# biuyq/CT-GAN

Hardware: AMD Instinct MI355X
Metric: img/s per (n_critic D + 1 G) step, CIFAR-10 ResNet (higher is better)
Workload: dtype f32

## Files before the change

ctgan_amd/csrc/fewch.hip:

```cpp
#include <hip/hip_runtime.h>
#include <stdint.h>
#include <stdlib.h>

#include "common.h"

namespace {

constexpr int NT = 256;

typedef float f32x2 __attribute__((ext_vector_type(2)));
__device__ __forceinline__ f32x2 pkfma(f32x2 a, f32x2 b, f32x2 c) { return __builtin_elementwise_fma(a, b, c); }
struct Acc4 { f32x2 lo, hi; };
__device__ __forceinline__ void fma4(float s, const Acc4& w, Acc4& a) {
    const f32x2 sv = {s, s};
    a.lo = pkfma(sv, w.lo, a.lo); a.hi = pkfma(sv, w.hi, a.hi);
}
__device__ __forceinline__ float4 to_f4(const Acc4& a) { return make_float4(a.lo.x, a.lo.y, a.hi.x, a.hi.y); }
__device__ __forceinline__ Acc4 to_acc(const float4& v) { Acc4 a; a.lo = f32x2{v.x, v.y}; a.hi = f32x2{v.z, v.w}; return a; }

template <int CTRL>
__device__ __forceinline__ float dpp_add(float v) {
    const int t = __builtin_amdgcn_update_dpp(0, __builtin_bit_cast(int, v), CTRL, 0xF, 0xF, true);
    return v + __builtin_bit_cast(float, t);
}
// ... 200 lines not shown
        const int c = i & 127, tj = i >> 7, j = tj % JS, t = tj / JS;
        wbuf[i] = p.w[p.w_off + (t / 3) * p.ws_r + (t % 3) * p.ws_s + (long long)c * p.ws_c + j * p.ws_j];
    }
    __builtin_amdgcn_s_waitcnt(0xF70 | 0);
    __syncthreads();
    f32x2 wlo[9][JS], whi[9][JS];
#pragma unroll
    for (int t = 0; t < 9; ++t)
#pragma unroll
        for (int j = 0; j < JS; ++j) {
            const float4 q = *reinterpret_cast<const float4*>(&wbuf[(t * JS + j) * 128 + l * 4]);
            wlo[t][j] = f32x2{q.x, q.y}; whi[t][j] = f32x2{q.z, q.w};
        }
    __builtin_amdgcn_sched_barrier(0);
    const int LPR = W >> 4;
    const float* img = p.x + (long long)n * p.xs_n;
    auto issue_row = [&](int r) {
        const int slot = (r + 1) & (RING_SLOTS - 1);
        if (r < 0 || r >= H) {
            for (int i = tid; i < W * 32; i += RING_NT) tile4[slot * slot_f4 + 32 + i] = zero4;
            return;
        }
        if (p.dbg & 1) return;
        const float* rowp = img + (long long)r * p.xs_h + (lane & 31) * 4;
        for (int c = 0; c < LPR; ++c) {
            const int chunk = c * 8 + wave;
            const unsigned dst = (unsigned)((slot * slot_f4 + (1 + 2 * chunk) * 32) * 16);
            lds_load16(rowp + (long long)(2 * chunk + (lane >> 5)) * p.xs_w, __builtin_amdgcn_readfirstlane(dst));
        }
    };
    const int last_row = p0 + np;
    for (int r = p0 - 1; r <= p0 + RING_AHEAD && r <= last_row; ++r) issue_row(r);

    for (int pp = 0; pp < np; ++pp) {
        const int prow = p0 + pp;
        if (prow + 1 + RING_AHEAD <= last_row) issue_row(prow + 1 + RING_AHEAD);
        int after = 0;
        for (int r = prow + 2; r <= prow + 1 + RING_AHEAD && r <= last_row; ++r) after += (r >= 0 && r < H) ? LPR : 0;
        wait_vmcnt(after);
        __syncthreads();
        const float4* r0 = tile4 + ((prow + 0) & (RING_SLOTS - 1)) * slot_f4;
        const float4* r1 = tile4 + ((prow + 1) & (RING_SLOTS - 1)) * slot_f4;
        const float4* r2 = tile4 + ((prow + 2) & (RING_SLOTS - 1)) * slot_f4;
        for (int qc = grp; qc < W && !(p.dbg & 2); qc += 16) {
            f32x2 acc[JS];
#pragma unroll
            for (int j = 0; j < JS; ++j) acc[j] = f32x2{0.f, 0.f};
#pragma unroll
            for (int r = 0; r < 3; ++r) {
                const float4* rowp = r == 0 ? r0 : (r == 1 ? r1 : r2);
#pragma unroll
                for (int s2 = 0; s2 < 3; ++s2) {
                    float4 xv = rowp[(qc + s2) * 32 + l];
                    if (p.relu_in) { xv.x = fmaxf(xv.x, 0.f); xv.y = fmaxf(xv.y, 0.f); xv.z = fmaxf(xv.z, 0.f); xv.w = fmaxf(xv.w, 0.f); }
                    const f32x2 xlo = {xv.x, xv.y}, xhi = {xv.z, xv.w};
#pragma unroll
                    for (int j = 0; j < JS; ++j) acc[j] = pkfma(xhi, whi[r * 3 + s2][j], pkfma(xlo, wlo[r * 3 + s2][j], acc[j]));
                }
            }
#pragma unroll
            for (int j = 0; j < JS; ++j) {
                float v = row16_sum(acc[j].x + acc[j].y);
                v += __shfl_xor(v, 16, 64);
                if (l == 0) obuf[(pp * JS + j) * W + qc] = v;
            }
        }
    }
    __syncthreads();
    for (int i = tid; i < np * JS * W; i += RING_NT) {
        const int qc = i % W, j = (i / W) % JS, pp = i / (W * JS);
        p.y[n * p.ys_n + (long long)j * p.ys_c + (long long)(p0 + pp) * p.ys_p + (long long)qc * p.ys_q] = obuf[i] + (p.bias ? p.bias[j] : 0.f);
    }
}


struct PXParams {
    const float* x; long long xs_n, xs_h, xs_w; int H, CM;
    float* y; long long ys_n, ys_c, ys_p, ys_q;
    const float* w; long long w_off, ws_r, ws_s, ws_c, ws_j;
    const float* bias;
    int relu_in, tiles;
    const float* bn_mean; const float* bn_rstd; const float* bn_scale; const float* bn_offset; int bn_per, tanh_out;
};
constexpr int PX_TH = 8, PX_W = 32, PX_CC = 32, PX_PS = 36, PX_NT = 256;
constexpr int PX_PIX = (PX_TH + 2) * (PX_W + 2);
constexpr int PX_F4 = PX_PIX * (PX_CC / 4);
constexpr int PX_PF = (PX_F4 + PX_NT - 1) / PX_NT;

template <int JS>
__global__ __launch_bounds__(PX_NT) void m2f_px_kernel(const PXParams p) {
    extern __shared__ __attribute__((aligned(16))) float tile[];
    float4* wl = reinterpret_cast<float4*>(tile + PX_PIX * PX_PS);
    constexpr int WF4 = 9 * (PX_CC / 4) * JS;
    static_assert(WF4 <= PX_NT, "one filter float4 per thread");
    const int tid = threadIdx.x;
    const int n = blockIdx.x / p.tiles, tb = blockIdx.x - n * p.tiles;
    const int p0 = tb * PX_TH;
    const int row = tid >> 5, col = tid & 31;
    const float* img = p.x + (long long)n * p.xs_n;
    float4 pf[PX_PF], wpf = make_float4(0.f, 0.f, 0.f, 0.f);
    auto fetch = [&](int chunk) {
        float4 mu = make_float4(0.f, 0.f, 0.f, 0.f), rs = mu, ga = mu, be = mu;
        if (p.bn_mean) {
            const int c = chunk * PX_CC + (tid & 7) * 4, g = n / p.bn_per;
            mu = *reinterpret_cast<const float4*>(p.bn_mean + (long long)g * p.CM + c); rs = *reinterpret_cast<const float4*>(p.bn_rstd + (long long)g * p.CM + c);
            ga = *reinterpret_cast<const float4*>(p.bn_scale + c); be = *reinterpret_cast<const float4*>(p.bn_offset + c);
        }
#pragma unroll
        for (int k = 0; k < PX_PF; ++k) {
            const int i = tid + k * PX_NT;
            const int pix = i >> 3, c4 = i & 7;
            const int tr = pix / (PX_W + 2), tw = pix - tr * (PX_W + 2);
            const int ih = p0 - 1 + tr, iw = tw - 1;
            float4 v = make_float4(0.f, 0.f, 0.f, 0.f);
            if (i < PX_F4 && (unsigned)ih < (unsigned)p.H && (unsigned)iw < (unsigned)PX_W) {
                v = *reinterpret_cast<const float4*>(img + (long long)ih * p.xs_h + (long long)iw * p.xs_w + chunk * PX_CC + c4 * 4);
                if (p.bn_mean) {
                    v.x = (v.x - mu.x) * rs.x * ga.x + be.x; v.y = (v.y - mu.y) * rs.y * ga.y + be.y;
                    v.z = (v.z - mu.z) * rs.z * ga.z + be.z; v.w = (v.w - mu.w) * rs.w * ga.w + be.w;
                }
            }
            pf[k] = v;
        }
        if (tid < WF4) {
            const int j = tid % JS, tc = tid / JS, c4 = tc & 7, t = tc >> 3;
            const float* q = p.w + p.w_off + (t / 3) * p.ws_r + (t % 3) * p.ws_s + (long long)(chunk * PX_CC + c4 * 4) * p.ws_c + j * p.ws_j;
            wpf = make_float4(q[0], q[p.ws_c], q[2 * p.ws_c], q[3 * p.ws_c]);
        }
    };
    auto stash = [&]() {
#pragma unroll
        for (int k = 0; k < PX_PF; ++k) {
            const int i = tid + k * PX_NT;
            if (i < PX_F4) {
                float4 v = pf[k];
                if (p.relu_in) { v.x = fmaxf(v.x, 0.f); v.y = fmaxf(v.y, 0.f); v.z = fmaxf(v.z, 0.f); v.w = fmaxf(v.w, 0.f); }
                *reinterpret_cast<float4*>(&tile[(i >> 3) * PX_PS + (i & 7) * 4]) = v;
            }
        }
        if (tid < WF4) wl[tid] = wpf;
    };
    f32x2 acc[JS][2];
#pragma unroll
    for (int j = 0; j < JS; ++j) { acc[j][0] = f32x2{0.f, 0.f}; acc[j][1] = f32x2{0.f, 0.f}; }
    const int nchunk = p.CM / PX_CC;
    fetch(0);
    for (int chunk = 0; chunk < nchunk; ++chunk) {
        __syncthreads();
        stash();
        __syncthreads();
        if (chunk + 1 < nchunk) fetch(chunk + 1);
#pragma unroll
        for (int t = 0; t < 9; ++t) {
            const int r = t / 3, s2 = t % 3;
            const float* xp = &tile[((row + r) * (PX_W + 2) + col + s2) * PX_PS];
#pragma unroll
            for (int c4 = 0; c4 < PX_CC / 4; ++c4) {
                const float4 xv = *reinterpret_cast<const float4*>(xp + c4 * 4);
#pragma unroll
                for (int j = 0; j < JS; ++j) {
                    const float4 wv = wl[(t * (PX_CC / 4) + c4) * JS + j];
                    acc[j][0] = pkfma(f32x2{xv.x, xv.y}, f32x2{wv.x, wv.y}, acc[j][0]);
                    acc[j][1] = pkfma(f32x2{xv.z, xv.w}, f32x2{wv.z, wv.w}, acc[j][1]);
                }
            }
        }
    }
    if (p0 + row < p.H) {
        const long long off = (long long)n * p.ys_n + (long long)(p0 + row) * p.ys_p + (long long)col * p.ys_q;
#pragma unroll
        for (int j = 0; j < JS; ++j) {
            const f32x2 a = acc[j][0] + acc[j][1];
            const float r = (a.x + a.y) + (p.bias ? p.bias[j] : 0.f);
            p.y[off + j * p.ys_c] = p.tanh_out ? tanhf(r) : r;
        }
    }
}

struct FWParams {
    const float* many; long long ms_n, ms_h, ms_w; int MH, MW, CM;
    const float* few; long long fs_n, fs_c, fs_h, fs_w; int FH, FW;
    int fst;
    int off_r[5], off_s[5];
    float* slab;
    int N, band, bands, total, relu_many, relu_few, few_in, with_bias, n_out, n_main;
    const float* many2; const float* few2; int N0, relu_many2, relu_few2, bias1, bias2;
};

template <int R, int S, int JS>
__global__ __launch_bounds__(NT) void fw_wgrad_kernel(const FWParams p) {
    extern __shared__ __attribute__((aligned(16))) float smem[];
    float4* tile = reinterpret_cast<float4*>(smem);
    const int tid = threadIdx.x;
    const int LPP = p.CM >> 2, GROUPS = NT / LPP;
    const int l = tid % LPP, grp = tid / LPP;
    int rmin = p.off_r[0], rmax = p.off_r[0], smin = p.off_s[0], smax = p.off_s[0];
#pragma unroll
    for (int r = 1; r < R; ++r) { rmin = min(rmin, p.off_r[r]); rmax = max(rmax, p.off_r[r]); }
#pragma unroll
    for (int s = 1; s < S; ++s) { smin = min(smin, p.off_s[s]); smax = max(smax, p.off_s[s]); }
    const int tw0 = smin, TW = (p.MW - 1) * p.fst + smax - smin + 1;

    Acc4 acc[R * S * JS];
#pragma unroll
    for (int i = 0; i < R * S * JS; ++i) { acc[i].lo = f32x2{0.f, 0.f}; acc[i].hi = f32x2{0.f, 0.f}; }
    float4 accb = make_float4(0.f, 0.f, 0.f, 0.f);

    for (int task = blockIdx.x; task < p.total; task += gridDim.x) {
        int n = task / p.bands;
        const int b = task - n * p.bands;
        const bool sg2 = n >= p.N0;
        const float* __restrict__ many = sg2 ? p.many2 : p.many;
        const float* __restrict__ few = sg2 ? p.few2 : p.few;
        const int relu_many = sg2 ? p.relu_many2 : p.relu_many, relu_few = sg2 ? p.relu_few2 : p.relu_few;
        const int seg_bias = sg2 ? p.bias2 : p.bias1;
        if (sg2) n -= p.N0;
        const int h0 = b * p.band, nh = min(p.band, p.MH - h0);
        const int tr0 = h0 * p.fst + rmin, TR = (nh - 1) * p.fst + rmax - rmin + 1;
        __syncthreads();
        for (int i = tid; i < TR * TW; i += NT) {
            const int tr = i / TW, tw = i - tr * TW;
            const int fh = tr0 + tr, fw = tw0 + tw;
            float v[4] = {0.f, 0.f, 0.f, 0.f};
            if ((unsigned)fh < (unsigned)p.FH && (unsigned)fw < (unsigned)p.FW) {
#pragma unroll
                for (int j = 0; j < JS; ++j) {
                    const float t = few[n * p.fs_n + j * p.fs_c + fh * p.fs_h + fw * p.fs_w];
                    v[j] = relu_few ? fmaxf(t, 0.f) : t;
                }
            }
            tile[i] = make_float4(v[0], v[1], v[2], v[3]);
        }
        __syncthreads();
        for (int hr = grp; hr < nh; hr += GROUPS) {
            const float* mrow = many + n * p.ms_n + (long long)(h0 + hr) * p.ms_h + l * 4;
            float4 mv = *reinterpret_cast<const float4*>(mrow);
            for (int w = 0; w < p.MW; ++w) {
                float4 cur = mv;
                if (w + 1 < p.MW) mv = *reinterpret_cast<const float4*>(mrow + (long long)(w + 1) * p.ms_w);
                if (relu_many) { cur.x = fmaxf(cur.x, 0.f); cur.y = fmaxf(cur.y, 0.f); cur.z = fmaxf(cur.z, 0.f); cur.w = fmaxf(cur.w, 0.f); }
                if (p.few_in && seg_bias) { accb.x += cur.x; accb.y += cur.y; accb.z += cur.z; accb.w += cur.w; }
                const Acc4 cm = to_acc(cur);
                const float4* trow = tile + (hr * p.fst - rmin) * TW + (w * p.fst - smin);
#pragma unroll
                for (int r = 0; r < R; ++r)
#pragma unroll
                    for (int s = 0; s < S; ++s) {
                        const float4 fv = trow[p.off_r[r] * TW + p.off_s[s]];
                        const float f[4] = {fv.x, fv.y, fv.z, fv.w};
#pragma unroll
                        for (int j = 0; j < JS; ++j) fma4(f[j], cm, acc[(r * S + s) * JS + j]);
                    }
                if (!p.few_in && seg_bias) {
                    const float4 fv = trow[0];
                    accb.x += fv.x; accb.y += fv.y; accb.z += fv.z; accb.w += fv.w;
                }
            }
        }
    }
// ... 221 lines not shown

template <typename KernelT>
int set_smem(KernelT k, size_t bytes) {
    if (bytes <= 48 * 1024) return 0;
    hipError_t e = hipFuncSetAttribute(reinterpret_cast<const void*>(k), hipFuncAttributeMaxDynamicSharedMemorySize, (int)bytes);
    if (e != hipSuccess) return ctgan_fail(CTGAN_E_LAUNCH, "hipFuncSetAttribute: %s", hipGetErrorString(e));
    return 0;
}

int tap_case(int R, int S, int few) {
    if (R == 3 && S == 3 && few == 3) return 1;
    if (R == 1 && S == 1 && few == 3) return 2;
    if (R == 5 && S == 5 && few == 1) return 3;
    if (R == 3 && S == 3 && few == 1) return 4;
    return 0;
}

int pick_band(int N, int rows, int unit, int min_tasks = 512) {
    int band = unit;
    while (band * 2 <= rows && (long long)N * ((rows + band * 2 - 1) / (band * 2)) >= min_tasks) band *= 2;
    return band;
}
#ifndef FW_TASKS
#define FW_TASKS 512
#endif

}

bool ctgan_fewch_handles(const ctgan_conv_desc* d) {
    if (d->x_up) return false;
    if (d->C <= 4 && tap_case(d->R, d->S, d->C) && many_ok(d->K)) return true;
    if (d->K <= 4 && d->stride == 1 && tap_case(d->R, d->S, d->K) && many_ok(d->C)) return true;
    return false;
}

static size_t f2m_tile_bytes(int band, int Q, int stride, int R, int S, int CS) {
    return (size_t)CS * ((band - 1) * stride + R) * ((Q - 1) * stride + S) * sizeof(float);
}
static int f2m_band(int N, int P, int Q, int stride, int R, int S, int CS) {
    int band = pick_band(N, P, 4);
    while (band > 4 && f2m_tile_bytes(band, Q, stride, R, S, CS) > 48 * 1024) band >>= 1;
    return f2m_tile_bytes(band, Q, stride, R, S, CS) > 150 * 1024 ? 0 : band;
}

static int launch_f2m(const F2MParams& p, int R, int S, int CS, hipStream_t st) {
    const int bands = (p.P + p.band - 1) / p.band;
    const size_t smem = f2m_tile_bytes(p.band, p.Q, p.stride, R, S, CS);
    const dim3 grid(p.N * bands), blk(NT);
    int rc = 0;
    switch (tap_case(R, S, CS)) {
        case 1: rc = set_smem(&f2m_kernel<3, 3, 3>, smem); if (!rc) hipLaunchKernelGGL((f2m_kernel<3, 3, 3>), grid, blk, smem, st, p); break;
        case 2: rc = set_smem(&f2m_kernel<1, 1, 3>, smem); if (!rc) hipLaunchKernelGGL((f2m_kernel<1, 1, 3>), grid, blk, smem, st, p); break;
        case 3: rc = set_smem(&f2m_kernel<5, 5, 1>, smem); if (!rc) hipLaunchKernelGGL((f2m_kernel<5, 5, 1>), grid, blk, smem, st, p); break;
        case 4: rc = set_smem(&f2m_kernel<3, 3, 1>, smem); if (!rc) hipLaunchKernelGGL((f2m_kernel<3, 3, 1>), grid, blk, smem, st, p); break;
        default: return ctgan_fail(CTGAN_E_UNSUPPORTED, "fewch f2m: taps");
    }
    if (rc) return rc;
    ctgan_set_last_symbol("f2m_kernel<%d, %d, %d>", R, S, CS);
    return ctgan_check_launch("fewch_f2m");
}

static bool m2f_ring_ok(const M2FParams& p, int R, int S) {
    return R == 3 && S == 3 && p.CM == 128 && p.pad_t == 1 && p.pad_l == 1 && (p.W == 32 || p.W == 16) && p.P == p.H && p.Q == p.W &&
           (p.xs_w % 4 == 0) && (p.xs_h % 4 == 0) && (p.xs_n % 4 == 0);
}

template <int JS>
static int launch_m2f_ring(M2FParams p, hipStream_t st) {
#ifndef M2F_DBG
#define M2F_DBG 0
#endif
    p.dbg = M2F_DBG;
    p.band = p.P >= 8 ? 8 : p.P;
    const int strips = (p.P + p.band - 1) / p.band;
    const size_t smem = (size_t)RING_SLOTS * (p.W + 2) * 128 * 4 + (size_t)p.band * JS * p.W * 4 + (size_t)9 * JS * 128 * 4;
    int rc = set_smem(&m2f_ring_kernel<JS>, smem);
    if (rc) return rc;
    hipLaunchKernelGGL((m2f_ring_kernel<JS>), dim3(p.N * strips), dim3(RING_NT), smem, st, p);
    ctgan_set_last_symbol("m2f_ring_kernel<%d>", JS);
    return ctgan_check_launch("fewch_m2f_ring");
}

static int g_m2f_px = 1;
extern "C" void ctgan_debug_m2f_px(int on) { g_m2f_px = on ? 1 : 0; }

static bool m2f_px_ok(const M2FParams& p, int R, int S, int JS) {
    return g_m2f_px && JS == 3 && R == 3 && S == 3 && p.pad_t == 1 && p.pad_l == 1 && p.W == PX_W && p.P == p.H && p.Q == p.W && p.CM % PX_CC == 0 &&
           (p.xs_w % 4 == 0) && (p.xs_h % 4 == 0) && (p.xs_n % 4 == 0);
}

static int launch_m2f_px(const M2FParams& m, hipStream_t st) {
    PXParams p;
    p.x = m.x; p.xs_n = m.xs_n; p.xs_h = m.xs_h; p.xs_w = m.xs_w; p.H = m.H; p.CM = m.CM;
    p.y = m.y; p.ys_n = m.ys_n; p.ys_c = m.ys_c; p.ys_p = m.ys_p; p.ys_q = m.ys_q;
    p.w = m.w; p.w_off = m.w_off; p.ws_r = m.ws_r; p.ws_s = m.ws_s; p.ws_c = m.ws_c; p.ws_j = m.ws_j;
    p.bias = m.bias; p.relu_in = m.relu_in;
    p.bn_mean = m.bn_mean; p.bn_rstd = m.bn_rstd; p.bn_scale = m.bn_scale; p.bn_offset = m.bn_offset; p.bn_per = m.bn_per; p.tanh_out = m.tanh_out;
    p.tiles = (m.H + PX_TH - 1) / PX_TH;
    const size_t smem = (size_t)PX_PIX * PX_PS * sizeof(float) + (size_t)9 * (PX_CC / 4) * 3 * sizeof(float4);
    int rc = set_smem(&m2f_px_kernel<3>, smem);
    if (rc) return rc;
    hipLaunchKernelGGL((m2f_px_kernel<3>), dim3(m.N * p.tiles), dim3(PX_NT), smem, st, p);
    ctgan_set_last_symbol("m2f_px_kernel<3>");
    return ctgan_check_launch("fewch_m2f_px");
}

static int launch_m2f(const M2FParams& p, int R, int S, int JS, hipStream_t st) {
    if (m2f_px_ok(p, R, S, JS)) return launch_m2f_px(p, st);
    if (m2f_ring_ok(p, R, S)) {
        if (JS == 3) return launch_m2f_ring<3>(p, st);
        if (JS == 1) return launch_m2f_ring<1>(p, st);
    }
    const int TR = p.band + R - 1, TW = p.Q + S - 1;
    const size_t smem = (size_t)TR * TW * p.CM * sizeof(float);
    const int grid = p.total < 512 ? p.total : 512;
    int rc = 0;
    switch (tap_case(R, S, JS)) {
        case 1: rc = set_smem(&m2f_kernel<3, 3, 3>, smem); if (!rc) hipLaunchKernelGGL((m2f_kernel<3, 3, 3>), dim3(grid), dim3(NT), smem, st, p); break;
        case 2: rc = set_smem(&m2f_kernel<1, 1, 3>, smem); if (!rc) hipLaunchKernelGGL((m2f_kernel<1, 1, 3>), dim3(grid), dim3(NT), smem, st, p); break;
        case 3: rc = set_smem(&m2f_kernel<5, 5, 1>, smem); if (!rc) hipLaunchKernelGGL((m2f_kernel<5, 5, 1>), dim3(grid), dim3(NT), smem, st, p); break;
        case 4: rc = set_smem(&m2f_kernel<3, 3, 1>, smem); if (!rc) hipLaunchKernelGGL((m2f_kernel<3, 3, 1>), dim3(grid), dim3(NT), smem, st, p); break;
        default: return ctgan_fail(CTGAN_E_UNSUPPORTED, "fewch m2f: taps");
    }
    if (rc) return rc;
    ctgan_set_last_symbol("m2f_kernel<%d, %d, %d>", R, S, JS);
    return ctgan_check_launch("fewch_m2f");
}

int ctgan_fewch_fwd(const ctgan_conv_desc* d, const float* x, const float* w, const float* bias, const float* mask, const float* resid,
                    float* y, int relu, int relu_in, hipStream_t st) {
    if (!ctgan_fewch_handles(d)) return 0;
    if (d->C <= 4) {
        if (d->ys[1] != 1 || (d->ys[0] | d->ys[2] | d->ys[3]) % 4 || !al16(y) || !al16(resid) || !al16(bias) || !al16(mask)) return 0;
        F2MParams p;
        p.x = x; p.xs_n = d->xs[0]; p.xs_c = d->xs[1]; p.xs_h = d->xs[2]; p.xs_w = d->xs[3]; p.H = d->H; p.W = d->W;
        p.y = y; p.ys_n = d->ys[0]; p.ys_p = d->ys[2]; p.ys_q = d->ys[3]; p.P = d->P; p.Q = d->Q; p.KM = d->K;
        p.w = w; p.w_off = 0; p.ws_r = (long long)d->S * d->C * d->K; p.ws_s = (long long)d->C * d->K; p.ws_c = d->K; p.ws_k = 1;
        p.bias = bias; p.resid = resid; p.mask = mask;
        p.N = d->N; p.stride = d->stride; p.pad_t = d->pad_t; p.pad_l = d->pad_l; p.relu = relu; p.relu_in = relu_in;
        p.band = f2m_band(d->N, d->P, d->Q, d->stride, d->R, d->S, d->C);
        if (!p.band) return 0;
        ctgan_set_last_kernel("fewch_f2m");
        const int rc = launch_f2m(p, d->R, d->S, d->C, st);
        return rc ? rc : 1;
    }
    if (resid || relu || mask) return 0;
    if (d->xs[1] != 1 || (d->xs[0] | d->xs[2] | d->xs[3]) % 4 || !al16(x)) return 0;
    M2FParams p; p.dbg = 0;
    p.x = x; p.xs_n = d->xs[0]; p.xs_h = d->xs[2]; p.xs_w = d->xs[3]; p.H = d->H; p.W = d->W; p.CM = d->C;
    p.y = y; p.ys_n = d->ys[0]; p.ys_c = d->ys[1]; p.ys_p = d->ys[2]; p.ys_q = d->ys[3]; p.P = d->P; p.Q = d->Q;
    p.w = w; p.w_off = 0; p.ws_r = (long long)d->S * d->C * d->K; p.ws_s = (long long)d->C * d->K; p.ws_c = d->K; p.ws_j = 1;
    p.bias = bias;
    p.N = d->N; p.pad_t = d->pad_t; p.pad_l = d->pad_l; p.relu_in = relu_in;
    p.band = 2;
    if ((size_t)(p.band + d->R - 1) * (d->Q + d->S - 1) * d->C * 4 > 150 * 1024) return 0;
    p.total = d->N * ((d->P + p.band - 1) / p.band);
    ctgan_set_last_kernel("fewch_m2f");
    const int rc = launch_m2f(p, d->R, d->S, d->K, st);
    return rc ? rc : 1;
}

int ctgan_fewch_fwd_bn(const ctgan_conv_desc* d, const float* x, const float* w, const float* bias, float* y, int relu_in, const float* mean,
                       const float* rstd, const float* scale, const float* offset, int groups, int tanh_out, hipStream_t st) {
    if (!ctgan_fewch_handles(d) || d->C <= 4 || groups <= 0 || d->N % groups) return 0;
    if (d->xs[1] != 1 || (d->xs[0] | d->xs[2] | d->xs[3]) % 4 || !al16(x) || !al16(mean) || !al16(rstd) || !al16(scale) || !al16(offset)) return 0;
    M2FParams p; p.dbg = 0;
    p.x = x; p.xs_n = d->xs[0]; p.xs_h = d->xs[2]; p.xs_w = d->xs[3]; p.H = d->H; p.W = d->W; p.CM = d->C;
    p.y = y; p.ys_n = d->ys[0]; p.ys_c = d->ys[1]; p.ys_p = d->ys[2]; p.ys_q = d->ys[3]; p.P = d->P; p.Q = d->Q;
    p.w = w; p.w_off = 0; p.ws_r = (long long)d->S * d->C * d->K; p.ws_s = (long long)d->C * d->K; p.ws_c = d->K; p.ws_j = 1;
    p.bias = bias;
    p.N = d->N; p.pad_t = d->pad_t; p.pad_l = d->pad_l; p.relu_in = relu_in;
    p.band = 2; p.total = d->N * ((d->P + 1) / 2);
    p.bn_mean = mean; p.bn_rstd = rstd; p.bn_scale = scale; p.bn_offset = offset; p.bn_per = d->N / groups; p.tanh_out = tanh_out;
    if (!m2f_px_ok(p, d->R, d->S, d->K)) return 0;
    ctgan_set_last_kernel("fewch_m2f(bn)");
    const int rc = launch_m2f_px(p, st);
    return rc ? rc : 1;
}

int ctgan_fewch_dgrad(const ctgan_conv_desc* d, const float* dy, const float* w, const float* bias, float* dx, hipStream_t st) {
    if (!ctgan_fewch_handles(d) || d->stride != 1) return 0;
    const long long tapR = (long long)d->S * d->C * d->K, tapS = (long long)d->C * d->K;
    const long long rot_off = (long long)(d->R - 1) * tapR + (long long)(d->S - 1) * tapS;
    if (d->C <= 4) {
        if (d->ys[1] != 1 || (d->ys[0] | d->ys[2] | d->ys[3]) % 4 || !al16(dy)) return 0;
        M2FParams p; p.dbg = 0;
        p.x = dy; p.xs_n = d->ys[0]; p.xs_h = d->ys[2]; p.xs_w = d->ys[3]; p.H = d->P; p.W = d->Q; p.CM = d->K;
        p.y = dx; p.ys_n = d->xs[0]; p.ys_c = d->xs[1]; p.ys_p = d->xs[2]; p.ys_q = d->xs[3]; p.P = d->H; p.Q = d->W;
        p.w = w; p.w_off = rot_off; p.ws_r = -tapR; p.ws_s = -tapS; p.ws_c = 1; p.ws_j = d->K;
        p.bias = bias;
        p.N = d->N; p.pad_t = d->R - 1 - d->pad_t; p.pad_l = d->S - 1 - d->pad_l; p.relu_in = 0;
        p.band = 2;
        if ((size_t)(p.band + d->R - 1) * (p.Q + d->S - 1) * p.CM * 4 > 150 * 1024) return 0;
        p.total = d->N * ((p.P + p.band - 1) / p.band);
        ctgan_set_last_kernel("fewch_m2f(dgrad)");
        const int rc = launch_m2f(p, d->R, d->S, d->C, st);
        return rc ? rc : 1;
    }
    if (d->xs[1] != 1 || (d->xs[0] | d->xs[2] | d->xs[3]) % 4 || !al16(dx) || !al16(bias)) return 0;
    F2MParams p;
    p.x = dy; p.xs_n = d->ys[0]; p.xs_c = d->ys[1]; p.xs_h = d->ys[2]; p.xs_w = d->ys[3]; p.H = d->P; p.W = d->Q;
    p.y = dx; p.ys_n = d->xs[0]; p.ys_p = d->xs[2]; p.ys_q = d->xs[3]; p.P = d->H; p.Q = d->W; p.KM = d->C;
    p.w = w; p.w_off = rot_off; p.ws_r = -tapR; p.ws_s = -tapS; p.ws_c = 1; p.ws_k = d->K;
    p.bias = bias; p.resid = nullptr; p.mask = nullptr;
    p.N = d->N; p.stride = 1; p.pad_t = d->R - 1 - d->pad_t; p.pad_l = d->S - 1 - d->pad_l; p.relu = 0; p.relu_in = 0;
    p.band = f2m_band(d->N, p.P, p.Q, 1, d->R, d->S, d->K);
    if (!p.band) return 0;
    ctgan_set_last_kernel("fewch_f2m(dgrad)");
    const int rc = launch_f2m(p, d->R, d->S, d->K, st);
    return rc ? rc : 1;
}

static void fw_plan(const ctgan_conv_desc* d, int* band, int* bands, int* n_main, int* n_out) {
    const int rows = d->C <= 4 ? d->P : d->H;
    const int cm = d->C <= 4 ? d->K : d->C;
    const int unit = NT / (cm / 4);
    *band = pick_band(d->N, rows, unit, FW_TASKS);
    *bands = (rows + *band - 1) / *band;
    *n_main = d->R * d->S * d->C * d->K;
    *n_out = *n_main + ((d->C <= 4 ? d->K : d->K) + 3) / 4 * 4;
}

size_t ctgan_fewch_wgrad_workspace(const ctgan_conv_desc* d) {
    if (!ctgan_fewch_handles(d)) return 0;
    int band, bands, n_main, n_out;
    fw_plan(d, &band, &bands, &n_main, &n_out);
    return (size_t)d->N * bands * n_out * sizeof(float);
}

int ctgan_fewch_wgrad(const ctgan_conv_desc* d, const float* x, const float* dy, float* dw, float* db, void* ws, size_t ws_bytes,
                      int relu_x, hipStream_t st) {
    return ctgan_fewch_wgrad2(d, x, dy, d->N, relu_x, db ? 1 : 0, nullptr, nullptr, 0, 0, 0, dw, db, ws, ws_bytes, st);
}

int ctgan_fewch_wgrad2(const ctgan_conv_desc* d0, const float* x, const float* dy, int N0, int relu_x, int bias0, const float* x1,
                       const float* dy1, int N1, int relu_x1, int bias1, float* dw, float* db, void* ws, size_t ws_bytes, hipStream_t st) {
    ctgan_conv_desc dd = *d0;
    dd.N = N0 + N1;
    const ctgan_conv_desc* d = &dd;
    if (!ctgan_fewch_handles(d)) return 0;
    if (N1 > 0 && (!x1 || !dy1 || !al16(x1) || !al16(dy1))) return 0;
    const bool few_in = d->C <= 4;
    FWParams p;
    p.N0 = N0; p.bias1 = bias0; p.bias2 = bias1;
    p.many2 = few_in ? dy1 : x1; p.few2 = few_in ? x1 : dy1;
    p.relu_many2 = few_in ? 0 : relu_x1; p.relu_few2 = few_in ? relu_x1 : 0;
    if (few_in) {
        if (d->ys[1] != 1 || (d->ys[0] | d->ys[2] | d->ys[3]) % 4 || !al16(dy)) return 0;
        p.many = dy; p.ms_n = d->ys[0]; p.ms_h = d->ys[2]; p.ms_w = d->ys[3]; p.MH = d->P; p.MW = d->Q; p.CM = d->K;
        p.few = x; p.fs_n = d->xs[0]; p.fs_c = d->xs[1]; p.fs_h = d->xs[2]; p.fs_w = d->xs[3]; p.FH = d->H; p.FW = d->W;
        p.fst = d->stride;
        for (int r = 0; r < d->R; ++r) p.off_r[r] = r - d->pad_t;
        for (int s = 0; s < d->S; ++s) p.off_s[s] = s - d->pad_l;
        p.relu_many = 0; p.relu_few = relu_x;
    } else {
        if (d->xs[1] != 1 || (d->xs[0] | d->xs[2] | d->xs[3]) % 4 || !al16(x)) return 0;
        p.many = x; p.ms_n = d->xs[0]; p.ms_h = d->xs[2]; p.ms_w = d->xs[3]; p.MH = d->H; p.MW = d->W; p.CM = d->C;
        p.few = dy; p.fs_n = d->ys[0]; p.fs_c = d->ys[1]; p.fs_h = d->ys[2]; p.fs_w = d->ys[3]; p.FH = d->P; p.FW = d->Q;
        p.fst = 1;
        for (int r = 0; r < d->R; ++r) p.off_r[r] = d->pad_t - r;
        for (int s = 0; s < d->S; ++s) p.off_s[s] = d->pad_l - s;
        p.relu_many = relu_x; p.relu_few = 0;
    }
    p.few_in = few_in ? 1 : 0; p.with_bias = db ? 1 : 0; p.N = d->N;
    fw_plan(d, &p.band, &p.bands, &p.n_main, &p.n_out);
    p.total = d->N * p.bands;
    const int blocks = p.total < 256 ? p.total : 256;
    const size_t need = (size_t)blocks * p.n_out * sizeof(float);
    if (!ws || ws_bytes < need) return ctgan_fail(CTGAN_E_BADARG, "conv2d_wgrad: workspace too small (%zu < %zu)", ws_bytes, need);
    p.slab = static_cast<float*>(ws);
    const int JS = few_in ? d->C : d->K;
    const int LPP = p.CM / 4, GROUPS = NT / LPP;
    int rspan = 0, sspan = 0;
    for (int r = 0; r < d->R; ++r) for (int r2 = 0; r2 < d->R; ++r2) if (p.off_r[r] - p.off_r[r2] > rspan) rspan = p.off_r[r] - p.off_r[r2];
    for (int s = 0; s < d->S; ++s) for (int s2 = 0; s2 < d->S; ++s2) if (p.off_s[s] - p.off_s[s2] > sspan) sspan = p.off_s[s] - p.off_s[s2];
    const size_t tile_b = (size_t)((p.band - 1) * p.fst + rspan + 1) * ((p.MW - 1) * p.fst + sspan + 1) * 16;
    const size_t red_b = (size_t)(GROUPS / 2) * LPP * (d->R * d->S * JS + 1) * 16;
// ... 53 lines not shown
```

ctgan_amd/kernels.py:

```python
import ctypes
import math
import os

import torch

from . import _lib
from ._lib import ConvDesc, I32x4, I64x4, check, lib

_ws_cache = {}

PROFILE = None


def _conv_flops(g, N):
    return 2.0 * N * g.P * g.Q * g.K * g.R * g.S * g.C


PROFILE_REPS = 1
PROFILE_CLOCKS = []
WGRAD_GROUP_EXTRA = 0


def _timed(g, N, launch):
    if PROFILE is None:
# ... 679 lines not shown
                    check(lib.ctgan_conv2d16_wgrad_group(arr3, len(x3), code, _ptr(ws3), ws3.numel(), 1 | (16 << which), _stream()), 'conv2d16_wgrad_group')
                    e1.record(st)
                mask = int(lib.ctgan_debug_last_wgrad_group_col_mask())
                flops = sum(f for k, f in enumerate(fl) if bool((mask >> k) & 1) == (which == 0))
                if flops:
                    PROFILE.append((last_kernel(), flops, e0, e1, 1, ('group', len(x3)), last_symbol()))
                    PROFILE_CLOCKS.append((last_symbol(), flops, probe))
            check(lib.ctgan_conv2d16_wgrad_group(arr3, len(x3), code, _ptr(ws3), ws3.numel(), 2, _stream()), 'conv2d16_wgrad_group')
        if not rest:
            return
        groups = [groups[i] for i in rest]
        arr, n = arr_r, len(rest)
    nb = lib.ctgan_conv2d_wgrad_group_workspace_bytes(arr, n)
    if nb == 0:
        raise NotImplementedError('conv2d_wgrad_group: unsupported group')
    ws = workspace(nb, dev)
    if PROFILE is None:
        check(lib.ctgan_conv2d_wgrad_group(arr, n, _ptr(ws), ws.numel(), _stream()), 'conv2d_wgrad_group')
        return
    st = torch.cuda.current_stream()
    for t in range(4):
        members = [i for i in range(n) if lib.ctgan_conv2d_wgrad_group_tile(ctypes.byref(arr[i])) == t]
        if not members:
            continue
        e0 = torch.cuda.Event(enable_timing=True)
        e1 = torch.cuda.Event(enable_timing=True)
        e0.record(st)
        for _ in range(PROFILE_REPS):
            check(lib.ctgan_conv2d_wgrad_group_ex(arr, n, _ptr(ws), ws.numel(), 1 | (16 << t), _stream()), 'conv2d_wgrad_group')
        e1.record(st)
        flops = sum(_conv_flops(groups[i][1], sum(sg[0].shape[0] for sg in groups[i][0])) for i in members)
        PROFILE.append((last_kernel(), flops, e0, e1, PROFILE_REPS, ('group', len(members)), last_symbol()))
    check(lib.ctgan_conv2d_wgrad_group_ex(arr, n, _ptr(ws), ws.numel(), 2, _stream()), 'conv2d_wgrad_group')


def im2col(x, g, cpad):
    _need_dev(x)
    N = x.shape[0]
    assert tuple(x.shape) == (N, g.C, g.H, g.W) and not g.x_up
    cols = empty_cl(N, cpad, g.P, g.Q, x.device)
    d = g.desc(N, x.stride(), cols.stride())
    check(lib.ctgan_im2col(ctypes.byref(d), _ptr(x), cpad, _ptr(cols), _stream()), 'im2col')
    return cols


def col2im(cols, g, N, out_strides=None):
    _need_dev(cols)
    cpad = cols.shape[1]
    assert tuple(cols.shape) == (N, cpad, g.P, g.Q) and cols.permute(0, 2, 3, 1).is_contiguous()
    if out_strides is None:
        dx = empty_cl(N, g.C, g.H, g.W, cols.device)
    else:
        dx = torch.empty_strided((N, g.C, g.H, g.W), out_strides, dtype=torch.float32, device=cols.device)
    d = g.desc(N, dx.stride(), cols.stride())
    check(lib.ctgan_col2im(ctypes.byref(d), _ptr(cols), cpad, _ptr(dx), _stream()), 'col2im')
    return dx


def last_kernel():
    return lib.ctgan_last_kernel().decode()


def last_symbol():
    return lib.ctgan_last_symbol().decode()


def debug_force_generic(on):
    lib.ctgan_debug_force_generic(1 if on else 0)


def debug_x3_halo_version(v):
    lib.ctgan_debug_x3_halo_version(int(v))


def debug_x3_s2fwd(on):
    lib.ctgan_debug_x3_s2fwd(2 if on == 2 else (1 if on else 0))


def debug_x3_s2halo(on):
    lib.ctgan_debug_x3_s2halo(1 if on else 0)


def debug_m2f_px(on):
    lib.ctgan_debug_m2f_px(1 if on else 0)


def debug_x3_hk(mode, max_wgs=0):
    lib.ctgan_debug_x3_hk(int(mode), int(max_wgs))


def debug_x3_halo_always(on):
    lib.ctgan_debug_x3_halo_always(1 if on else 0)


if os.environ.get('CTGAN_X3_HK') is not None:
    _hk = os.environ['CTGAN_X3_HK'].split(':')
    debug_x3_hk(int(_hk[0]), int(_hk[1]) if len(_hk) > 1 else 0)
if os.environ.get('CTGAN_M2F_PX') == '0':
    debug_m2f_px(False)
if os.environ.get('CTGAN_X3_S2HALO') == '0':
    debug_x3_s2halo(False)
if os.environ.get('CTGAN_X3_S2DGRAD_SF') == '-1':
    lib.ctgan_debug_x3_s2dgrad_sf(-1)
if os.environ.get('CTGAN_X3_S2FWD') in ('0', '2'):
    debug_x3_s2fwd(int(os.environ['CTGAN_X3_S2FWD']))


def debug_last_wgrad_group_kinds():
    return int(lib.ctgan_debug_last_wgrad_group_kinds())


class ClockProbe:
    _side = None

    def __init__(self, cap_ms=50.0):
        self.cap_ticks = int(cap_ms * 1e5)

    def __enter__(self):
        dev = torch.device('cuda', torch.cuda.current_device())
        if ClockProbe._side is None:
            ClockProbe._side = torch.cuda.Stream()
        self.flag = torch.zeros(1, dtype=torch.int32, device=dev)
        self.out = torch.zeros(5, dtype=torch.int64, device=dev)
        ev = torch.cuda.Event()
        ev.record(torch.cuda.current_stream())
        ClockProbe._side.wait_event(ev)
        check(lib.ctgan_debug_clock_probe(_ptr(self.flag), self.cap_ticks, _ptr(self.out), ctypes.c_void_p(ClockProbe._side.cuda_stream)), 'clock_probe')
        return self

    def __exit__(self, *exc):
        self.flag.fill_(1)
        return False

    def result(self):
        r0, s0, r1, s1, seen = [int(v) for v in self.out.cpu().tolist()]
        dr = max(r1 - r0, 1)
        return 100.0 * (s1 - s0) / dr, dr / 100.0, bool(seen)

    def mhz(self):
        return self.result()[0]


def colsum_channels(gy):
    _need_dev(gy)
    N, K, P, Q = gy.shape
    if not gy.permute(0, 2, 3, 1).is_contiguous():
        gy = to_channels_last(gy)
    out = torch.empty(K, dtype=torch.float32, device=gy.device)
    rows = N * P * Q
    nb = lib.ctgan_colsum_workspace_bytes(rows, K)
    ws = workspace(nb, gy.device)
    check(lib.ctgan_colsum(_ptr(gy), rows, K, K, _ptr(out), _ptr(ws), ws.numel(), _stream()), 'colsum')
    return out


def _ew_out(x):
    if not is_dense(x):
        raise ValueError('elementwise kernels need dense tensors')
    return empty_like_dense(x)


def lrelu_fwd(x, alpha):
    _need_dev(x)
    y = _ew_out(x)
    check(lib.ctgan_lrelu_fwd(_ptr(x), _ptr(y), x.numel(), alpha, _stream()), 'lrelu_fwd')
    return y

# ... 1487 lines not shown
```

Measured before the change: 25570.

## Restructure m2f_px conv to split channels across waves with row-strip register reuse

Reworks the few-output-channel 3x3 conv kernel so each wave handles a quarter of the channel quads of a chunk, while each thread computes a 4-row strip of outputs. Each loaded input float4 is reused across the three filter rows, which cuts LDS reads per FMA. Partial sums from the four waves are reduced through shared memory at the end, and blocks start at staggered channel chunks to spread global traffic. It also adds an opt-in mode (flag value 2) that sends more conv shapes to this kernel, but that mode is off by default. The cost is more accumulator registers, with waves_per_eu capped at 2, plus an extra reduction pass through shared memory.

```diff
diff --git a/ctgan_amd/csrc/fewch.hip b/ctgan_amd/csrc/fewch.hip
--- a/ctgan_amd/csrc/fewch.hip
+++ b/ctgan_amd/csrc/fewch.hip
@@ -306,38 +306,34 @@
     int relu_in, tiles;
     const float* bn_mean; const float* bn_rstd; const float* bn_scale; const float* bn_offset; int bn_per, tanh_out;
 };
-constexpr int PX_TH = 8, PX_W = 32, PX_CC = 32, PX_PS = 36, PX_NT = 256;
-constexpr int PX_PIX = (PX_TH + 2) * (PX_W + 2);
-constexpr int PX_F4 = PX_PIX * (PX_CC / 4);
-constexpr int PX_PF = (PX_F4 + PX_NT - 1) / PX_NT;
-
-template <int JS>
-__global__ __launch_bounds__(PX_NT) void m2f_px_kernel(const PXParams p) {
-    extern __shared__ __attribute__((aligned(16))) float tile[];
-    float4* wl = reinterpret_cast<float4*>(tile + PX_PIX * PX_PS);
-    constexpr int WF4 = 9 * (PX_CC / 4) * JS;
-    static_assert(WF4 <= PX_NT, "one filter float4 per thread");
-    const int tid = threadIdx.x;
-    const int n = blockIdx.x / p.tiles, tb = blockIdx.x - n * p.tiles;
-    const int p0 = tb * PX_TH;
-    const int row = tid >> 5, col = tid & 31;
-    const float* img = p.x + (long long)n * p.xs_n;
-    float4 pf[PX_PF], wpf = make_float4(0.f, 0.f, 0.f, 0.f);
-    auto fetch = [&](int chunk) {
+constexpr int PX_W = 32, PX_CC = 32, PX_PS = 36, PX_NT = 256, PX_COLS = PX_W + 2, PX_WAVES = PX_NT / 64;
+constexpr int PX_TH = 8, PX_SP = 4;
+
+template <int JS, int TH, int NTHR>
+struct PXStage {
+    static constexpr int PIX = (TH + 2) * PX_COLS;
+    static constexpr int F4 = PIX * (PX_CC / 4);
+    static constexpr int PF = (F4 + NTHR - 1) / NTHR;
+    static constexpr int WF4 = 9 * (PX_CC / 4) * JS, WPF = (WF4 + NTHR - 1) / NTHR;
+    static constexpr int REGION = PIX * PX_PS + WF4 * 4;
+    static_assert(NTHR % (PX_CC / 4) == 0, "a thread's channel quad is the same for all its items: one set of BN coefficients per chunk");
+    float4 pf[PF], wpf[WPF];
+
+    __device__ __forceinline__ void fetch(const PXParams& p, const float* img, int n, int p0, int chunk, int t) {
         float4 mu = make_float4(0.f, 0.f, 0.f, 0.f), rs = mu, ga = mu, be = mu;
         if (p.bn_mean) {
-            const int c = chunk * PX_CC + (tid & 7) * 4, g = n / p.bn_per;
+            const int c = chunk * PX_CC + (t & 7) * 4, g = n / p.bn_per;
             mu = *reinterpret_cast<const float4*>(p.bn_mean + (long long)g * p.CM + c); rs = *reinterpret_cast<const float4*>(p.bn_rstd + (long long)g * p.CM + c);
             ga = *reinterpret_cast<const float4*>(p.bn_scale + c); be = *reinterpret_cast<const float4*>(p.bn_offset + c);
         }
 #pragma unroll
-        for (int k = 0; k < PX_PF; ++k) {
-            const int i = tid + k * PX_NT;
+        for (int k = 0; k < PF; ++k) {
+            const int i = t + k * NTHR;
             const int pix = i >> 3, c4 = i & 7;
-            const int tr = pix / (PX_W + 2), tw = pix - tr * (PX_W + 2);
+            const int tr = pix / PX_COLS, tw = pix - tr * PX_COLS;
             const int ih = p0 - 1 + tr, iw = tw - 1;
             float4 v = make_float4(0.f, 0.f, 0.f, 0.f);
-            if (i < PX_F4 && (unsigned)ih < (unsigned)p.H && (unsigned)iw < (unsigned)PX_W) {
+            if (i < F4 && (unsigned)ih < (unsigned)p.H && (unsigned)iw < (unsigned)PX_W) {
                 v = *reinterpret_cast<const float4*>(img + (long long)ih * p.xs_h + (long long)iw * p.xs_w + chunk * PX_CC + c4 * 4);
                 if (p.bn_mean) {
                     v.x = (v.x - mu.x) * rs.x * ga.x + be.x; v.y = (v.y - mu.y) * rs.y * ga.y + be.y;
@@ -346,59 +342,117 @@
             }
             pf[k] = v;
         }
-        if (tid < WF4) {
-            const int j = tid % JS, tc = tid / JS, c4 = tc & 7, t = tc >> 3;
-            const float* q = p.w + p.w_off + (t / 3) * p.ws_r + (t % 3) * p.ws_s + (long long)(chunk * PX_CC + c4 * 4) * p.ws_c + j * p.ws_j;
-            wpf = make_float4(q[0], q[p.ws_c], q[2 * p.ws_c], q[3 * p.ws_c]);
-        }
-    };
-    auto stash = [&]() {
-#pragma unroll
-        for (int k = 0; k < PX_PF; ++k) {
-            const int i = tid + k * PX_NT;
-            if (i < PX_F4) {
+#pragma unroll
+        for (int k = 0; k < WPF; ++k) {
+            const int i = t + k * NTHR;
+            wpf[k] = make_float4(0.f, 0.f, 0.f, 0.f);
+            if (i < WF4) {
+                const int j = i % JS, tc = i / JS, c4 = tc & 7, tap = tc >> 3;
+                const float* q = p.w + p.w_off + (tap / 3) * p.ws_r + (tap % 3) * p.ws_s + (long long)(chunk * PX_CC + c4 * 4) * p.ws_c + j * p.ws_j;
+                wpf[k] = make_float4(q[0], q[p.ws_c], q[2 * p.ws_c], q[3 * p.ws_c]);
+            }
+        }
+    }
+    __device__ __forceinline__ void stash(const PXParams& p, float* region, int t) const {
+        float4* wl = reinterpret_cast<float4*>(region + PIX * PX_PS);
+#pragma unroll
+        for (int k = 0; k < PF; ++k) {
+            const int i = t + k * NTHR;
+            if (i < F4) {
                 float4 v = pf[k];
                 if (p.relu_in) { v.x = fmaxf(v.x, 0.f); v.y = fmaxf(v.y, 0.f); v.z = fmaxf(v.z, 0.f); v.w = fmaxf(v.w, 0.f); }
-                *reinterpret_cast<float4*>(&tile[(i >> 3) * PX_PS + (i & 7) * 4]) = v;
-            }
-        }
-        if (tid < WF4) wl[tid] = wpf;
-    };
-    f32x2 acc[JS][2];
-#pragma unroll
-    for (int j = 0; j < JS; ++j) { acc[j][0] = f32x2{0.f, 0.f}; acc[j][1] = f32x2{0.f, 0.f}; }
+                *reinterpret_cast<float4*>(&region[(i >> 3) * PX_PS + (i & 7) * 4]) = v;
+            }
+        }
+#pragma unroll
+        for (int k = 0; k < WPF; ++k) {
+            const int i = t + k * NTHR;
+            if (i < WF4) wl[i] = wpf[k];
+        }
+    }
+};
+
+template <int JS, int SP, int NQ, int PIX>
+__device__ __forceinline__ void px_strip_fma(const float* region, int r0, int col, int q0, f32x2 (&acc)[SP][JS][2]) {
+    const float4* wl = reinterpret_cast<const float4*>(region + PIX * PX_PS);
+#pragma unroll
+    for (int q = 0; q < NQ; ++q) {
+        const int c4 = q0 + q;
+#pragma unroll
+        for (int s2 = 0; s2 < 3; ++s2) {
+            float4 xv[SP + 2];
+#pragma unroll
+            for (int i = 0; i < SP + 2; ++i) xv[i] = *reinterpret_cast<const float4*>(&region[((r0 + i) * PX_COLS + col + s2) * PX_PS + c4 * 4]);
+#pragma unroll
+            for (int r = 0; r < 3; ++r)
+#pragma unroll
+                for (int j = 0; j < JS; ++j) {
+                    const float4 wv = wl[((r * 3 + s2) * (PX_CC / 4) + c4) * JS + j];
+#pragma unroll
+                    for (int i = 0; i < SP; ++i) {
+                        acc[i][j][0] = pkfma(f32x2{xv[i + r].x, xv[i + r].y}, f32x2{wv.x, wv.y}, acc[i][j][0]);
+                        acc[i][j][1] = pkfma(f32x2{xv[i + r].z, xv[i + r].w}, f32x2{wv.z, wv.w}, acc[i][j][1]);
+                    }
+                }
+        }
+    }
+}
+
+template <int JS, int SP, int TH>
+__device__ __forceinline__ void px_finish(const PXParams& p, float* part, const f32x2 (&acc)[SP][JS][2], int wave, int sr, int col, int n, int p0) {
+    constexpr int TP = TH * PX_W;
+    static_assert(TP <= PX_NT && PX_WAVES == 4, "one tile pixel per thread, four partial sums");
+#pragma unroll
+    for (int i = 0; i < SP; ++i)
+#pragma unroll
+        for (int j = 0; j < JS; ++j) {
+            const f32x2 a = acc[i][j][0] + acc[i][j][1];
+            part[(wave * JS + j) * TP + (sr * SP + i) * PX_W + col] = a.x + a.y;
+        }
+    __syncthreads();
+    const int t = threadIdx.x, row = t >> 5, c = t & 31;
+    if (t < TP && p0 + row < p.H) {
+        const long long off = (long long)n * p.ys_n + (long long)(p0 + row) * p.ys_p + (long long)c * p.ys_q;
+#pragma unroll
+        for (int j = 0; j < JS; ++j) {
+            float r = (part[j * TP + t] + part[(JS + j) * TP + t]) + (part[(2 * JS + j) * TP + t] + part[(3 * JS + j) * TP + t]);
+            r += p.bias ? p.bias[j] : 0.f;
+            p.y[off + j * p.ys_c] = p.tanh_out ? tanhf(r) : r;
+        }
+    }
+}
+
+template <int JS>
+__global__ __launch_bounds__(PX_NT) __attribute__((amdgpu_waves_per_eu(2))) void m2f_px_kernel(const PXParams p) {
+    extern __shared__ __attribute__((aligned(16))) float tile[];
+    const int tid = threadIdx.x, lane = tid & 63, wave = __builtin_amdgcn_readfirstlane(tid >> 6);
+    const int sr = lane >> 5, col = lane & 31;
+    const int n = blockIdx.x / p.tiles, tb = blockIdx.x - n * p.tiles;
+    const float* img = p.x + (long long)n * p.xs_n;
     const int nchunk = p.CM / PX_CC;
-    fetch(0);
+    using Stage = PXStage<JS, PX_TH, PX_NT>;
+    static_assert(PX_WAVES * JS * PX_TH * PX_W <= Stage::REGION, "the partial sums fit the staged chunk's place");
+    static_assert((PX_CC / 4) % PX_WAVES == 0, "channel quads per wave");
+    constexpr int NQ = (PX_CC / 4) / PX_WAVES;
+    const int p0 = tb * PX_TH;
+    f32x2 acc[PX_SP][JS][2];
+#pragma unroll
+    for (int i = 0; i < PX_SP; ++i)
+#pragma unroll
+        for (int j = 0; j < JS; ++j) { acc[i][j][0] = f32x2{0.f, 0.f}; acc[i][j][1] = f32x2{0.f, 0.f}; }
+    Stage st;
+    int cur = tb % nchunk;
+    st.fetch(p, img, n, p0, cur, tid);
     for (int chunk = 0; chunk < nchunk; ++chunk) {
         __syncthreads();
-        stash();
-        __syncthreads();
-        if (chunk + 1 < nchunk) fetch(chunk + 1);
-#pragma unroll
-        for (int t = 0; t < 9; ++t) {
-            const int r = t / 3, s2 = t % 3;
-            const float* xp = &tile[((row + r) * (PX_W + 2) + col + s2) * PX_PS];
-#pragma unroll
-            for (int c4 = 0; c4 < PX_CC / 4; ++c4) {
-                const float4 xv = *reinterpret_cast<const float4*>(xp + c4 * 4);
-#pragma unroll
-                for (int j = 0; j < JS; ++j) {
-                    const float4 wv = wl[(t * (PX_CC / 4) + c4) * JS + j];
-                    acc[j][0] = pkfma(f32x2{xv.x, xv.y}, f32x2{wv.x, wv.y}, acc[j][0]);
-                    acc[j][1] = pkfma(f32x2{xv.z, xv.w}, f32x2{wv.z, wv.w}, acc[j][1]);
-                }
-            }
-        }
-    }
-    if (p0 + row < p.H) {
-        const long long off = (long long)n * p.ys_n + (long long)(p0 + row) * p.ys_p + (long long)col * p.ys_q;
-#pragma unroll
-        for (int j = 0; j < JS; ++j) {
-            const f32x2 a = acc[j][0] + acc[j][1];
-            const float r = (a.x + a.y) + (p.bias ? p.bias[j] : 0.f);
-            p.y[off + j * p.ys_c] = p.tanh_out ? tanhf(r) : r;
-        }
-    }
+        st.stash(p, tile, tid);
+        __syncthreads();
+        cur = cur + 1 == nchunk ? 0 : cur + 1;
+        if (chunk + 1 < nchunk) st.fetch(p, img, n, p0, cur, tid);
+        px_strip_fma<JS, PX_SP, NQ, Stage::PIX>(tile, sr * PX_SP, col, wave * NQ, acc);
+    }
+    __syncthreads();
+    px_finish<JS, PX_SP, PX_TH>(p, tile, acc, wave, sr, col, n, p0);
 }
 
 struct FWParams {
@@ -786,7 +840,7 @@
 }
 
 static int g_m2f_px = 1;
-extern "C" void ctgan_debug_m2f_px(int on) { g_m2f_px = on ? 1 : 0; }
+extern "C" void ctgan_debug_m2f_px(int on) { g_m2f_px = on == 2 ? 2 : (on ? 1 : 0); }
 
 static bool m2f_px_ok(const M2FParams& p, int R, int S, int JS) {
     return g_m2f_px && JS == 3 && R == 3 && S == 3 && p.pad_t == 1 && p.pad_l == 1 && p.W == PX_W && p.P == p.H && p.Q == p.W && p.CM % PX_CC == 0 &&
@@ -801,7 +855,7 @@
     p.bias = m.bias; p.relu_in = m.relu_in;
     p.bn_mean = m.bn_mean; p.bn_rstd = m.bn_rstd; p.bn_scale = m.bn_scale; p.bn_offset = m.bn_offset; p.bn_per = m.bn_per; p.tanh_out = m.tanh_out;
     p.tiles = (m.H + PX_TH - 1) / PX_TH;
-    const size_t smem = (size_t)PX_PIX * PX_PS * sizeof(float) + (size_t)9 * (PX_CC / 4) * 3 * sizeof(float4);
+    const size_t smem = sizeof(float) * PXStage<3, PX_TH, PX_NT>::REGION;
     int rc = set_smem(&m2f_px_kernel<3>, smem);
     if (rc) return rc;
     hipLaunchKernelGGL((m2f_px_kernel<3>), dim3(m.N * p.tiles), dim3(PX_NT), smem, st, p);
@@ -831,9 +885,12 @@
     return ctgan_check_launch("fewch_m2f");
 }
 
+static bool px_only_width(const ctgan_conv_desc* d, int many) { return g_m2f_px == 2 && !d->x_up && d->stride == 1 && many > 4 && many % PX_CC == 0; }
+
 int ctgan_fewch_fwd(const ctgan_conv_desc* d, const float* x, const float* w, const float* bias, const float* mask, const float* resid,
                     float* y, int relu, int relu_in, hipStream_t st) {
-    if (!ctgan_fewch_handles(d)) return 0;
+    const bool any_kernel = ctgan_fewch_handles(d);
+    if (!any_kernel && !(d->K <= 4 && px_only_width(d, d->C))) return 0;
     if (d->C <= 4) {
         if (d->ys[1] != 1 || (d->ys[0] | d->ys[2] | d->ys[3]) % 4 || !al16(y) || !al16(resid) || !al16(bias) || !al16(mask)) return 0;
         F2MParams p;
@@ -859,6 +916,7 @@
     p.band = 2;
     if ((size_t)(p.band + d->R - 1) * (d->Q + d->S - 1) * d->C * 4 > 150 * 1024) return 0;
     p.total = d->N * ((d->P + p.band - 1) / p.band);
+    if (!any_kernel && !m2f_px_ok(p, d->R, d->S, d->K)) return 0;
     ctgan_set_last_kernel("fewch_m2f");
     const int rc = launch_m2f(p, d->R, d->S, d->K, st);
     return rc ? rc : 1;
@@ -883,7 +941,8 @@
 }
 
 int ctgan_fewch_dgrad(const ctgan_conv_desc* d, const float* dy, const float* w, const float* bias, float* dx, hipStream_t st) {
-    if (!ctgan_fewch_handles(d) || d->stride != 1) return 0;
+    const bool any_kernel = ctgan_fewch_handles(d);
+    if (d->stride != 1 || (!any_kernel && !(d->C <= 4 && px_only_width(d, d->K)))) return 0;
     const long long tapR = (long long)d->S * d->C * d->K, tapS = (long long)d->C * d->K;
     const long long rot_off = (long long)(d->R - 1) * tapR + (long long)(d->S - 1) * tapS;
     if (d->C <= 4) {
@@ -897,6 +956,7 @@
         p.band = 2;
         if ((size_t)(p.band + d->R - 1) * (p.Q + d->S - 1) * p.CM * 4 > 150 * 1024) return 0;
         p.total = d->N * ((p.P + p.band - 1) / p.band);
+        if (!any_kernel && !m2f_px_ok(p, d->R, d->S, d->C)) return 0;
         ctgan_set_last_kernel("fewch_m2f(dgrad)");
         const int rc = launch_m2f(p, d->R, d->S, d->C, st);
         return rc ? rc : 1;
diff --git a/ctgan_amd/kernels.py b/ctgan_amd/kernels.py
--- a/ctgan_amd/kernels.py
+++ b/ctgan_amd/kernels.py
@@ -785,7 +785,7 @@
 
 
 def debug_m2f_px(on):
-    lib.ctgan_debug_m2f_px(1 if on else 0)
+    lib.ctgan_debug_m2f_px(int(on))
 
 
 def debug_x3_hk(mode, max_wgs=0):
```

Result: no change. 25630, median of 6 (+0.2%).
